# IML-DKFZ/values

Hardware: AMD Instinct MI355X
Metric: uncertainty-volumes/sec (64^3, T=10 MC-dropout) (higher is better)
Workload: dtype f32; 1 GPU; C2: 64^3 1-channel volumes, UNet3D(initial_filter_size=8, 2 classes), T=10 MC-dropout passes + fused softmax/entropy/MI/variance/argmax reduction; dropout=hash bit generator, new seed every step, weights=torch default init, seed 123

## Files before the change

include/values_amd.h:

```cpp
#ifndef VALUES_AMD_H
#define VALUES_AMD_H

#include <stddef.h>
#include <stdint.h>

#ifdef __cplusplus
extern "C" {
#endif

typedef void* vx_stream_t;

enum {
  VX_OK = 0,
  VX_E_NULL = -1,
  VX_E_SHAPE = -2,
  VX_E_DTYPE = -3,
  VX_E_WORKSPACE = -4,
  VX_E_ALIGN = -5
};

enum { VX_F32 = 0, VX_F64 = 1 };
enum { VX_ACT_NONE = 0, VX_ACT_LRELU = 1 , VX_ACT_RELU = 2 };
enum { VX_DROP_NONE = 0, VX_DROP_HASH = 1, VX_DROP_MASK = 2 };

// ... 107 lines not shown
  const float* acc_in;
  int32_t acc_pitch;
  int32_t out_planar, in_planar;
  int32_t products;
} vx_conv3d_args;
int64_t vx_conv3d_upfused_packed_floats(void);
int vx_pack_conv3d_upfused(const float* w1_torch, const float* b1, const float* up_w_torch, const float* up_b, float* packed,
                           vx_stream_t stream);
int vx_conv3d_k3_prologue_ok(int D, int H, int W, int Cin, int Cout);
int vx_conv3d_k3_upfuse_ok(int D, int H, int W, int Cin, int Cout);
int64_t vx_convT_zc16_packed_floats(void);
int vx_pack_convT_zc16(const float* w_torch , float* packed, vx_stream_t stream);
int vx_conv3d_k3_skip_prologue_ok(int D, int H, int W, int Cin, int Cout, int xblk);
int vx_conv3d_k3_acc_ok(int D, int H, int W, int Cin, int Cout);
int vx_conv3d_k3_planar_ok(int D, int H, int W, int Cin, int Cout);
int vx_conv3d_k3_poolfuse_ok(int D, int H, int W, int Cin, int Cout);
int vx_conv3d_k3_presplit_ok(int D, int H, int W, int Cin, int Cout);
int vx_conv3d_k3_poolfin_ok(int Cin, int Cout);
int vx_prenorm_split(float* x, const float* mean, const float* rstd, int N, int64_t nvox, float scale, vx_stream_t stream);
int vx_pool_finish(const float* pool_raw, const uint32_t* pool_flags, const float* mean, const float* rstd, float* out,
                   int out_pitch, int N, int64_t voxels_per_sample, int drop_scale2, vx_stream_t stream);
int vx_pool_finish_z(const float* pool_raw, const uint32_t* pool_flags, const float* mean, const float* rstd, float* out,
                     int out_pitch, int N, int Dp, int64_t plane_voxels, int drop_scale2, vx_stream_t stream);
int vx_conv3d_k3_pool_layout(int D, int H, int W, int Cin, int Cout);
int vx_conv3d_k3_tiles(int D, int H, int W);
int vx_conv3d_k3_tiles_for(int D, int H, int W, int Cout);
int vx_conv3d_k3(const vx_conv3d_args* a, vx_stream_t stream);
int vx_conv3d_k3_head_fusable(int Cin, int Cout);

int vx_conv3d_k3_c1_tiles(int D, int H, int W);
int vx_conv3d_k3_c1(const float* in, const float* w_torch , const float* bias, float* out,
                    int out_pitch, int N, int D, int H, int W, int Cout, int repeat, const int32_t* src,
                    const int32_t* flip, float* stats_partial, vx_stream_t stream);

int vx_pack_input_cl8(const float* in, float* out, int N, int Cin, int D, int H, int W, int repeat, const int32_t* src,
                      const int32_t* flip, vx_stream_t stream);

int vx_instnorm_finalize(const float* stats_partial, int N, int ntiles, int C, int64_t nvox, float eps,
                         float* mean, float* rstd, vx_stream_t stream);

typedef struct vx_norm_args {
  const float* x; int32_t x_pitch;
  const float* mean; const float* rstd;
  float* out; int32_t out_pitch, out_coff;
  float* pool_out; int32_t pool_pitch;
  int32_t N, D, H, W, C;
  int32_t act, drop_mode; uint32_t drop_seed, drop_layer; const uint8_t* drop_mask;
  int32_t out_xblk, out_half;
  int32_t x_xblk, x_half;
  const uint32_t* seed_dev;
  uint32_t* range_flag;
} vx_norm_args;
int vx_norm_act_drop_pool(const vx_norm_args* a, vx_stream_t stream);
typedef struct vx_stat_src {
  const float* stats_partial; int32_t tiles; float eps; int64_t count;
  float* mean_out; float* rstd_out;
} vx_stat_src;
int vx_norm_act_drop_pool_stats(const vx_norm_args* a, const vx_stat_src* st, vx_stream_t stream);
int vx_prenorm_split_stats(float* x, const vx_stat_src* st, int N, int64_t nvox, float scale, vx_stream_t stream);
int vx_zero(void* p, int64_t bytes, vx_stream_t stream);
int vx_pool_finish_z_stats(const float* pool_raw, const uint32_t* pool_flags, const vx_stat_src* st, float* out, int out_pitch,
                           int N, int Dp, int64_t plane_voxels, int drop_scale2, vx_stream_t stream);
int vx_norm_act_drop_pool_bcast(const vx_norm_args* a, int x_repeat, vx_stream_t stream);

typedef struct vx_convT_args {
  const float* in; int32_t in_pitch;
// ... 348 lines not shown
```

values_amd/_lib.py:

```python
from __future__ import annotations

import ctypes as C
import os

_HERE = os.path.dirname(os.path.abspath(__file__))
LIB_PATH = os.environ.get("VX_LIB_PATH") or os.path.join(_HERE, "libvalues_amd.so")

VX_F32, VX_F64 = 0, 1
VX_ACT_NONE, VX_ACT_LRELU, VX_ACT_RELU = 0, 1, 2
VX_DROP_NONE, VX_DROP_HASH, VX_DROP_MASK = 0, 1, 2

_p = C.c_void_p
_i = C.c_int
_i32 = C.c_int32
_u32 = C.c_uint32
_i64 = C.c_int64


class ConvArgs(C.Structure):
    _fields_ = [("in_", _p), ("w_packed", _p), ("bias", _p), ("out", _p),
                ("in_pitch", _i32), ("out_pitch", _i32), ("out_coff", _i32),
                ("N", _i32), ("D", _i32), ("H", _i32), ("W", _i32), ("Cin", _i32), ("Cout", _i32),
                ("act", _i32), ("drop_mode", _i32), ("drop_seed", _u32), ("drop_layer", _u32),
                ("drop_mask", _p), ("stats_partial", _p), ("in_xblk", _i32), ("w_family", _i32),
# ... 203 lines not shown
    "vx_unc_stats_accumulate": (_i, [_p, _i, _i, _i, _i64, _p, _p]),
    "vx_unc_stats_finalize": (_i, [_p, _i, _i, _i, _i64, _p, _p, _p, _p, _p, _p]),
    "vx_softmax_planar": (_i, [_p, _i64, _i, _i64, _p, _p]),
    "vx_one_minus_msr": (_i, [_p, _i, _i, _i64, _p, _p]),
    "vx_one_minus_msr_batched_workspace_bytes": (_i64, [_i, _i]),
    "vx_one_minus_msr_batched": (_i, [C.POINTER(MsrItem), _i, C.POINTER(_p), _i, _p, _i64, _p]),
    "vx_conv3d_k3_packed_floats": (_i64, [_i, _i]),
    "vx_pack_conv3d_k3": (_i, [_p, _p, _i, _i, _p]),
    "vx_convT_k2s2_packed_floats": (_i64, [_i, _i]),
    "vx_pack_convT_k2s2": (_i, [_p, _p, _i, _i, _p]),
    "vx_conv3d_k3_tiles": (_i, [_i, _i, _i]),
    "vx_conv3d_k3_tiles_for": (_i, [_i, _i, _i, _i]),
    "vx_conv3d_k3_head_fusable": (_i, [_i, _i]),
    "vx_conv3d_k3_prologue_ok": (_i, [_i, _i, _i, _i, _i]),
    "vx_conv3d_k3_upfuse_ok": (_i, [_i, _i, _i, _i, _i]),
    "vx_conv3d_k3_poolfuse_ok": (_i, [_i, _i, _i, _i, _i]),
    "vx_conv3d_k3_presplit_ok": (_i, [_i, _i, _i, _i, _i]),
    "vx_conv3d_k3_poolfin_ok": (_i, [_i, _i]),
    "vx_conv3d_upfused_packed_floats": (_i64, []),
    "vx_pack_conv3d_upfused": (_i, [_p, _p, _p, _p, _p, _p]),
    "vx_pool_finish": (_i, [_p, _p, _p, _p, _p, _i, _i, _i64, _i, _p]),
    "vx_pool_finish_z": (_i, [_p, _p, _p, _p, _p, _i, _i, _i, _i64, _i, _p]),
    "vx_conv3d_k3_pool_layout": (_i, [_i, _i, _i, _i, _i]),
    "vx_conv3d_k3_skip_prologue_ok": (_i, [_i, _i, _i, _i, _i, _i]),
    "vx_conv3d_k3_acc_ok": (_i, [_i, _i, _i, _i, _i]),
    "vx_conv3d_k3_planar_ok": (_i, [_i, _i, _i, _i, _i]),
    "vx_convT_zc16_packed_floats": (_i64, []),
    "vx_pack_convT_zc16": (_i, [_p, _p, _p]),
    "vx_prenorm_split": (_i, [_p, _p, _p, _i, _i64, C.c_float, _p]),
    "vx_zero": (_i, [_p, _i64, _p]),
    "vx_conv3d_k3": (_i, [C.POINTER(ConvArgs), _p]),
    "vx_conv3d_k3_c1_tiles": (_i, [_i, _i, _i]),
    "vx_conv3d_k3_c1": (_i, [_p, _p, _p, _p, _i, _i, _i, _i, _i, _i, _i, _p, _p, _p, _p]),
    "vx_pack_input_cl8": (_i, [_p, _p, _i, _i, _i, _i, _i, _i, _p, _p, _p]),
    "vx_instnorm_finalize": (_i, [_p, _i, _i, _i, _i64, C.c_float, _p, _p, _p]),
    "vx_norm_act_drop_pool": (_i, [C.POINTER(NormArgs), _p]),
    "vx_norm_act_drop_pool_bcast": (_i, [C.POINTER(NormArgs), _i, _p]),
    "vx_norm_act_drop_pool_stats": (_i, [C.POINTER(NormArgs), C.POINTER(StatSrc), _p]),
    "vx_prenorm_split_stats": (_i, [_p, C.POINTER(StatSrc), _i, _i64, C.c_float, _p]),
    "vx_pool_finish_z_stats": (_i, [_p, _p, C.POINTER(StatSrc), _p, _i, _i, _i, _i64, _i, _p]),
    "vx_convT_k2s2": (_i, [C.POINTER(ConvTArgs), _p]),
    "vx_conv1x1_ncdhw": (_i, [_p, _i, _p, _p, _p, _i, _i, _i, _i, _i, _i, _p, _p, _p]),
    "vx_unet3d_workspace_bytes": (C.c_size_t, [_i, _i, _i, _i, _i]),
    "vx_unet3d_forward": (_i, [C.POINTER(UNet3DWeights), C.POINTER(UNet3DRun), _p]),
    "vx_unet3d_forward_profiled": (_i, [C.POINTER(UNet3DWeights), C.POINTER(UNet3DRun), _p, _i, C.POINTER(C.c_float),
                                        C.POINTER(C.c_char_p), C.POINTER(_i)]),
    "vx_softmax_accumulate": (_i, [_p, _i, _i, _i, _i, _i, _i, _p, _p, _p, _i, _i, _i, _i, _p]),
    "vx_aleatoric_sample": (_i, [_p, _p, _u32, _i, _i, _i, _i64, _p, _p, _p]),
    "vx_colorize_u8": (_i, [_p, _p, _i64, _p, _i, _p, _p]),
    "vx_fuse_sum": (_i, [C.POINTER(FuseArgs), _p]),
    "vx_tta_views_2d": (_i, [_p, _i, _p, _p, C.POINTER(C.c_float), C.POINTER(C.c_float), C.c_float, _i, _i, _i, _i,
                             C.POINTER(C.c_int32), _p, _p]),
    "vx_count_nonzero_batched_workspace_bytes": (_i64, [_i]),
    "vx_count_nonzero_batched": (_i, [C.POINTER(CountItem), _i, _p, _p, _i64, _p]),
    "vx_select_segments_workspace_bytes": (_i64, [_i]),
    "vx_select_segments": (_i, [C.POINTER(SelectItem), _i, _i64, _p, _p, _p, _i64, _p]),
    "vx_mask_agreement": (_i, [_p, _i, _i, _i64, _p, _p]),
    "vx_mask_agreement_batched": (_i, [_p, _i, _i, _i, _i64, _i, _p, _p]),
    "vx_soft_metric_workspace_bytes": (_i64, [_i, _i]),
    "vx_soft_metric_sums": (_i, [_p, _p, _i, _i, _i64, _p, _p, _p]),
    "vx_soft_metric_batched_workspace_bytes": (_i64, [_i, _i, _i, _i64]),
    "vx_soft_metric_sums_batched": (_i, [_p, _p, _i, _i, _i, _i64, _p, _p, _p]),
    "vx_ssn2d_lowres": (_i, [_p, _i, _p, _i, _p, _u32, _i, _i64, _i, _i, _i, _p, _p, _p]),
    "vx_ssn2d_add_diag": (_i, [_p, _p, _p, _u32, _i, _i, _i64, C.c_float, _p]),
    "vx_softmax_variance": (_i, [_p, _i, _i, _i, _i, _i64, _p, _p]),
    "vx_ssn_sample": (_i, [_p, _p, _p, _u32, _i, _i, _i, _i, _i64, C.c_float, _p, _p]),
# ... 155 lines not shown
```

values_amd/csrc/conv3d_c1.hip:

```cpp
#include "s16_common.h"

template <int COUT>
__global__ __launch_bounds__(256) void conv3d_k3_c1_kernel(const float* __restrict__ in, const float* __restrict__ w,
                                                           const float* __restrict__ bias,
                                                           float* __restrict__ out, int out_pitch, int N, int D, int H, int W,
                                                           int repeat, const int32_t* __restrict__ src,
                                                           const int32_t* __restrict__ flip, float* __restrict__ stats_partial,
                                                           int tiles_x, int tiles_y, int tiles_z) {
  constexpr int TX = 64, TY = 4, TZ = 4;
  constexpr int HX = TX + 2, HY = TY + 2, HZ = TZ + 2;
  __shared__ float s_in[HZ * HY * HX];
  __shared__ __attribute__((aligned(16))) float s_w[27 * COUT];
  __shared__ float s_red[16][COUT][2];

  const int tid = threadIdx.x;
  int t = blockIdx.x;
  const int tx = t % tiles_x; t /= tiles_x;
  const int ty = t % tiles_y; t /= tiles_y;
  const int tz = t % tiles_z; t /= tiles_z;
  const int n = t;
  const int v = src ? src[n] : n / repeat;
  const int f = flip ? flip[n] : 0;
  const int x0 = tx * TX, y0 = ty * TY, z0 = tz * TZ;
  const float* in_v = in + (size_t)v * D * H * W;

  for (int idx = tid; idx < HZ * HY * HX; idx += 256) {
    const int hx = idx % HX, hy = (idx / HX) % HY, hz = idx / (HX * HY);
    int gx = x0 + hx - 1, gy = y0 + hy - 1, gz = z0 + hz - 1;
    float val = 0.f;
    if ((unsigned)gx < (unsigned)W && (unsigned)gy < (unsigned)H && (unsigned)gz < (unsigned)D) {
      if (f & 1) gz = D - 1 - gz;
      if (f & 2) gy = H - 1 - gy;
      if (f & 4) gx = W - 1 - gx;
      val = in_v[((size_t)gz * H + gy) * W + gx];
    }
    s_in[idx] = val;
  }
  for (int idx = tid; idx < 27 * COUT; idx += 256) {
    const int co = idx % COUT, tap = idx / COUT;
    s_w[idx] = w[co * 27 + tap];
  }
  __syncthreads();

  const int lx = tid % TX, ly = tid / TX;
  float acc[TZ][COUT];
#pragma unroll
  for (int z = 0; z < TZ; ++z)
#pragma unroll
    for (int c = 0; c < COUT; ++c) acc[z][c] = bias[c];
#pragma unroll 1
  for (int kk = 0; kk < 9; ++kk) {
    const int ky = kk / 3, kx = kk - 3 * ky;
    float wk[3][COUT];
#pragma unroll
    for (int kz = 0; kz < 3; ++kz)
#pragma unroll
      for (int c = 0; c < COUT; c += 4) {
        const f32x4 w4 = *reinterpret_cast<const f32x4*>(&s_w[(kz * 9 + kk) * COUT + c]);
        wk[kz][c] = w4[0]; wk[kz][c + 1] = w4[1]; wk[kz][c + 2] = w4[2]; wk[kz][c + 3] = w4[3];
      }
    const float* sp = s_in + (ly + ky) * HX + lx + kx;
#pragma unroll
    for (int p = 0; p < HZ; ++p) {
      const float xv = sp[p * HY * HX];
#pragma unroll
      for (int z = 0; z < TZ; ++z) {
        const int kz = p - z;
        if (kz < 0 || kz > 2) continue;
#pragma unroll
        for (int c = 0; c < COUT; ++c) acc[z][c] = fmaf(wk[kz][c], xv, acc[z][c]);
      }
    }
  }

  const int gx = x0 + lx, gy = y0 + ly;
  float ssum[COUT], ssq[COUT];
#pragma unroll
  for (int c = 0; c < COUT; ++c) { ssum[c] = 0.f; ssq[c] = 0.f; }
#pragma unroll
  for (int z = 0; z < TZ; ++z) {
    const int gz = z0 + z;
    const bool valid = gx < W && gy < H && gz < D;
    if (valid) {
      float* o = out + (((size_t)(n * D + gz) * H + gy) * W + gx) * out_pitch;
#pragma unroll
      for (int c = 0; c < COUT; c += 4)
        *reinterpret_cast<f32x4*>(o + c) = (f32x4){acc[z][c], acc[z][c + 1], acc[z][c + 2], acc[z][c + 3]};
#pragma unroll
      for (int c = 0; c < COUT; ++c) { ssum[c] += acc[z][c]; ssq[c] = fmaf(acc[z][c], acc[z][c], ssq[c]); }
    }
  }
  if (stats_partial) {
    const int lane = tid & 63, wave = tid >> 6;
#pragma unroll
    for (int c = 0; c < COUT; ++c) {
      float s = ssum[c], q = ssq[c];
#pragma unroll
      for (int rot = 8; rot >= 1; rot >>= 1) { s += vx_row_ror(s, rot); q += vx_row_ror(q, rot); }
      if ((lane & 15) == 0) { s_red[wave * 4 + (lane >> 4)][c][0] = s; s_red[wave * 4 + (lane >> 4)][c][1] = q; }
    }
    __syncthreads();
    if (tid < COUT) {
      float s = 0.f, q = 0.f;
#pragma unroll
      for (int wv = 0; wv < 16; ++wv) { s += s_red[wv][tid][0]; q += s_red[wv][tid][1]; }
      const int ntiles = tiles_x * tiles_y * tiles_z;
      const int tile = blockIdx.x % ntiles;
      float* dst = stats_partial + (((size_t)n * ntiles + tile) * COUT + tid) * 2;
      dst[0] = s;
      dst[1] = q;
    }
  }
}

extern "C" int vx_conv3d_k3_c1_tiles(int D, int H, int W) { return ((W + 63) / 64) * ((H + 3) / 4) * ((D + 3) / 4); }

extern "C" int vx_conv3d_k3_c1(const float* in, const float* w_torch, const float* bias, float* out, int out_pitch,
                               int N, int D, int H, int W, int Cout, int repeat, const int32_t* src,
                               const int32_t* flip, float* stats_partial, vx_stream_t stream) {
  if (!in || !w_torch || !bias || !out) VX_FAIL(VX_E_NULL, "vx_conv3d_k3_c1: null pointer");
  if (N <= 0 || D <= 0 || H <= 0 || W <= 0) VX_FAIL(VX_E_SHAPE, "vx_conv3d_k3_c1: empty tensor");
  if (repeat <= 0) VX_FAIL(VX_E_SHAPE, "vx_conv3d_k3_c1: repeat must be >= 1");
  if (out_pitch < Cout || out_pitch % 4 || !vx_aligned16(out)) VX_FAIL(VX_E_ALIGN, "vx_conv3d_k3_c1: out pitch/alignment");
  const int tiles_x = (W + 63) / 64, tiles_y = (H + 3) / 4, tiles_z = (D + 3) / 4;
  dim3 grid((unsigned)(tiles_x * tiles_y * tiles_z * N));
  hipStream_t s = (hipStream_t)stream;
#define VX_C1(CO)                                                                                                  \
  vx_note_kernel("conv3d_k3_c1_kernel<" #CO ">");                                                                  \
  hipLaunchKernelGGL(conv3d_k3_c1_kernel<CO>, grid, dim3(256), 0, s, in, w_torch, bias, out, out_pitch, N, D, H, W, \
                     repeat, src, flip, stats_partial, tiles_x, tiles_y, tiles_z)
  switch (Cout) {
    case 8: VX_C1(8); break;
    case 16: VX_C1(16); break;
    case 32: VX_C1(32); break;
    default: VX_FAIL(VX_E_SHAPE, "vx_conv3d_k3_c1: Cout=%d unsupported (8, 16, 32)", Cout);
  }
#undef VX_C1
  VX_CHECK_LAUNCH("vx_conv3d_k3_c1");
  return VX_OK;
}

__global__ __launch_bounds__(256) void pack_input_cl8_kernel(const float* __restrict__ in, float* __restrict__ out, int N, int Cin,
                                                             int D, int H, int W, int repeat, const int32_t* __restrict__ src,
                                                             const int32_t* __restrict__ flip) {
  const int64_t nvox = (int64_t)D * H * W, total = (int64_t)N * nvox;
  for (int64_t i = blockIdx.x * (int64_t)blockDim.x + threadIdx.x; i < total; i += (int64_t)gridDim.x * blockDim.x) {
    const int n = (int)(i / nvox);
    const int64_t v = i - (int64_t)n * nvox;
    int x = (int)(v % W), y = (int)((v / W) % H), z = (int)(v / ((int64_t)W * H));
    const int vol = src ? src[n] : n / repeat;
    const int fl = flip ? flip[n] : 0;
    if (fl & 1) z = D - 1 - z;
    if (fl & 2) y = H - 1 - y;
    if (fl & 4) x = W - 1 - x;
    const float* p = in + ((size_t)vol * Cin) * nvox + ((size_t)z * H + y) * W + x;
    f32x4 lo = {0.f, 0.f, 0.f, 0.f}, hi = {0.f, 0.f, 0.f, 0.f};
#pragma unroll
    for (int c = 0; c < 4; ++c) {
      if (c < Cin) lo[c] = p[(size_t)c * nvox];
      if (c + 4 < Cin) hi[c] = p[(size_t)(c + 4) * nvox];
    }
    reinterpret_cast<f32x4*>(out + (size_t)i * 8)[0] = lo;
    reinterpret_cast<f32x4*>(out + (size_t)i * 8)[1] = hi;
  }
}

extern "C" int vx_pack_input_cl8(const float* in, float* out, int N, int Cin, int D, int H, int W, int repeat,
                                 const int32_t* src, const int32_t* flip, vx_stream_t stream) {
  if (!in || !out) VX_FAIL(VX_E_NULL, "vx_pack_input_cl8: null pointer");
  if (N <= 0 || D <= 0 || H <= 0 || W <= 0 || repeat <= 0) VX_FAIL(VX_E_SHAPE, "vx_pack_input_cl8: empty tensor");
  if (Cin < 1 || Cin > 8) VX_FAIL(VX_E_SHAPE, "vx_pack_input_cl8: in_channels %d (1 .. 8)", Cin);
  if (!vx_aligned16(out)) VX_FAIL(VX_E_ALIGN, "vx_pack_input_cl8: output alignment");
// ... 9 lines not shown
```

values_amd/csrc/lib.cpp:

```cpp
#include <stdarg.h>
#include <stdio.h>
#include <stdlib.h>
#include <string.h>

#include "../../include/values_amd.h"

static thread_local char g_err[512] = "";

void vx_set_error(const char* fmt, ...) {
  va_list ap;
  va_start(ap, fmt);
  vsnprintf(g_err, sizeof(g_err), fmt, ap);
  va_end(ap);
}

static thread_local const char* g_last_kernel = nullptr;
void vx_note_kernel(const char* name) { g_last_kernel = name; }
const char* vx_last_kernel() { return g_last_kernel; }
const char* vx_kname(const char* fmt, ...) {
  char buf[256];
  va_list ap;
  va_start(ap, fmt);
  vsnprintf(buf, sizeof(buf), fmt, ap);
  va_end(ap);
// ... 26 lines not shown
  g_cfg.no_head_fusion = env_int("VX_NO_HEAD_FUSION", 0);
  g_cfg.s16_no_upfuse = env_int("VX_S16_NO_UPFUSE", 0);
  g_cfg.s16_no_poolfuse = env_int("VX_S16_NO_POOLFUSE", 0);
  g_cfg.storage16 = env_int("VX_STORAGE16", 0);
  g_cfg.s16_generic = env_int("VX_S16_GENERIC", 0);
  g_cfg.s16_no_zc16 = env_int("VX_S16_NO_ZC16", 0);
  g_cfg.s16_no_halves = env_int("VX_S16_NO_HALVES", 0);
  g_cfg.s16_no_deep = env_int("VX_S16_NO_DEEP", 0);
  g_cfg.s16_no_l1dma = env_int("VX_S16_NO_L1DMA", 0);
  g_cfg.c2s_no_wide = env_int("VX_C2S_NO_WIDE", 0);
  g_cfg.c2s_no_oct = env_int("VX_C2S_NO_OCT", 0);
}

const vx_config& vx_cfg() {
  std::call_once(g_cfg_once, cfg_from_env);
  return g_cfg;
}

extern "C" int vx_get_config(vx_config* out) {
  if (!out) { vx_set_error("vx_get_config: null"); return VX_E_NULL; }
  *out = vx_cfg();
  return VX_OK;
}

extern "C" int vx_set_config(const vx_config* cfg) {
  if (!cfg) { vx_set_error("vx_set_config: null"); return VX_E_NULL; }
  if (cfg->conv_fp32 < 0 || cfg->conv_fp32 > 2) { vx_set_error("vx_set_config: conv_fp32 %d", cfg->conv_fp32); return VX_E_DTYPE; }
  (void)vx_cfg();
  g_cfg = *cfg;
  return VX_OK;
}

extern "C" const char* vx_last_kernel_name(void) { return g_last_kernel ? g_last_kernel : ""; }
extern "C" int vx_version(void) { return 840;  }
extern "C" const char* vx_last_error_string(void) { return g_err; }
```

values_amd/csrc/unet3d_forward.hip:

```cpp
#include "common.h"
#include <stdlib.h>

extern "C" int vx_conv3d_k3_c1_tiles(int D, int H, int W);

namespace {
struct Level { int D, H, W, C; int64_t nvox; };

struct Plan {
  Level lv[5];
  float *A[4], *B[4], *CAT[4], *P[5], *C0, *C1;
  float *stats, *mean, *rstd;
  float *mean0, *rstd0;
  float *meanS[4], *rstdS[4];
  size_t bytes;
};

static size_t align_up(size_t v) { return (v + 255) & ~(size_t)255; }

static void make_plan(Plan& p, int N, int D, int H, int W, int F, char* base) {
  size_t off = 0;
  auto carve = [&](size_t floats) {
    float* q = base ? (float*)(base + off) : nullptr;
    off += align_up(floats * sizeof(float));
    return q;
  };
  for (int l = 0; l < 5; ++l) {
    p.lv[l].D = D >> l; p.lv[l].H = H >> l; p.lv[l].W = W >> l; p.lv[l].C = F << l;
    p.lv[l].nvox = (int64_t)p.lv[l].D * p.lv[l].H * p.lv[l].W;
  }
  for (int l = 0; l < 4; ++l) {
    const size_t e = (size_t)N * p.lv[l].nvox * p.lv[l].C;
    p.A[l] = carve(e);
    p.B[l] = carve(e);
    p.CAT[l] = carve(2 * e);
  }
  p.P[0] = nullptr;
// ... 43 lines not shown
thread_local char g_prof_labels[Prof::MAXL][192];
}

#define VX_TRY(expr)            \
  do {                          \
    int rc_ = (expr);           \
    if (rc_ != VX_OK) return rc_; \
  } while (0)

#define VX_STEP(label, expr)                                                       \
  do {                                                                             \
    Prof* pf_ = g_prof;                                                            \
    if (pf_ && pf_->n < Prof::MAXL) { vx_note_kernel(nullptr); (void)hipEventRecord(pf_->ev[2 * pf_->n], pf_->s); }  \
    int rc_ = (expr);                                                              \
    if (rc_ != VX_OK) return rc_;                                                  \
    if (pf_ && pf_->n < Prof::MAXL) {                                              \
      (void)hipEventRecord(pf_->ev[2 * pf_->n + 1], pf_->s);                             \
      pf_->kernel[pf_->n] = vx_last_kernel();                                      \
      pf_->name[pf_->n++] = (label);                                               \
    }                                                                              \
  } while (0)

namespace {
int xblk_of(int W) { return W % 4 == 0 ? 4 : (W % 2 == 0 ? 2 : 1); }

struct Flow {
  bool inorm;
  int ich;
  int rep;
  bool shared;
  bool fuse_head;
  bool pre[4];
  bool presplit;
  bool skip_raw[4];
  bool pooled[4];
  bool poolfin1;
  bool halves[4];
  bool fuse_up;
  bool fuse_up1;
  bool split_out[4];
  bool planar1;
  bool st16;
  int products_c12, products_e11, products_e12;
};

Flow decide_flow(const vx_unet3d_weights* w, const vx_unet3d_run* r, const Plan& p) {
  const vx_config& cfg = vx_cfg();
  const int F = w->F, dm = r->drop_mode;
  const Level* lv = p.lv;
  const bool hashed = dm != VX_DROP_MASK;
  Flow f = {};
  f.inorm = !w->no_instancenorm;
  f.ich = w->in_channels > 1 ? w->in_channels : 1;
  f.rep = r->repeat > 0 ? r->repeat : 1;
  f.shared = !r->src && !r->flip && f.rep > 1 && r->N % f.rep == 0;
  f.fuse_head = w->num_classes <= 4 && vx_conv3d_k3_head_fusable(F, F) && !cfg.no_head_fusion;
  f.pre[0] = hashed && !cfg.s16_no_prenorm && F == 8 && f.inorm && vx_conv3d_k3_prologue_ok(lv[0].D, lv[0].H, lv[0].W, F, F);
  for (int l = 1; l < 4; ++l)
    f.pre[l] = f.inorm && hashed && !cfg.s16_no_prenorm && vx_conv3d_k3_prologue_ok(lv[l].D, lv[l].H, lv[l].W, lv[l].C, lv[l].C);
  f.presplit = f.shared && f.pre[0] && vx_conv3d_k3_presplit_ok(lv[0].D, lv[0].H, lv[0].W, F, F);
  f.skip_raw[0] = f.pre[0] && cfg.s16_skip_raw && vx_conv3d_k3_prologue_ok(lv[0].D, lv[0].H, lv[0].W, 2 * F, F);
  f.pooled[0] = f.skip_raw[0] && vx_conv3d_k3_poolfuse_ok(lv[0].D, lv[0].H, lv[0].W, F, F);
  f.poolfin1 = f.pooled[0] && vx_conv3d_k3_poolfin_ok(F, 2 * F);
  for (int l = 1; l < 4; ++l) {
    const Level& L = lv[l];
    f.skip_raw[l] = f.pooled[l] = f.inorm && hashed && !cfg.s16_no_prenorm && cfg.s16_skip_raw &&
                                  vx_conv3d_k3_pool_layout(L.D, L.H, L.W, L.C, L.C) == 2 &&
                                  vx_conv3d_k3_skip_prologue_ok(L.D, L.H, L.W, 2 * L.C, L.C, xblk_of(L.W));
  }
  f.halves[1] = f.skip_raw[1] && lv[1].C == 16 && w->split_w[0] && w->split_w[1] && !cfg.s16_no_halves &&
                w->split_family == vx_conv3d_k3_family(16, 16) && vx_conv3d_k3_acc_ok(lv[1].D, lv[1].H, lv[1].W, 16, 16);
  f.fuse_up = hashed && F == 8 && vx_conv3d_k3_upfuse_ok(lv[0].D, lv[0].H, lv[0].W, 2 * F, F);
  f.fuse_up1 = f.halves[1] && w->up3_zc16 && hashed && vx_conv3d_k3_upfuse_ok(lv[1].D, lv[1].H, lv[1].W, 16, 16) == 2;
  f.split_out[1] = f.fuse_up;
  f.split_out[2] = f.fuse_up1;
  f.planar1 = f.fuse_up1 && !cfg.s16_no_l1dma && vx_conv3d_k3_planar_ok(lv[1].D, lv[1].H, lv[1].W, 16, 16);
  f.st16 = cfg.storage16 && dm == VX_DROP_HASH && F == 8 && f.fuse_head && cfg.conv_fp32 == 0 &&
           vx_conv3d_k3_prologue_ok(lv[0].D, lv[0].H, lv[0].W, F, F);
  const bool one = f.st16 && cfg.storage16 == 2;
  f.products_c12 = one && f.presplit && f.pooled[0];
  f.products_e11 = one && f.skip_raw[0] && f.fuse_up && w->up_fused;
  f.products_e12 = one;
  return f;
}
}

extern "C" int vx_unet3d_forward(const vx_unet3d_weights* w, const vx_unet3d_run* r, vx_stream_t stream) {
  if (!w || !r) VX_FAIL(VX_E_NULL, "vx_unet3d_forward: null argument");
  if (!r->x || !r->logits || !r->workspace) VX_FAIL(VX_E_NULL, "vx_unet3d_forward: null tensor/workspace");
  const int N = r->N, D = r->D, H = r->H, W = r->W, F = w->F, NC = w->num_classes;
  if (N <= 0 || D <= 0 || H <= 0 || W <= 0) VX_FAIL(VX_E_SHAPE, "vx_unet3d_forward: empty batch");
  if (D % 16 || H % 16 || W % 16)
    VX_FAIL(VX_E_SHAPE, "vx_unet3d_forward: spatial size (%d,%d,%d) must be divisible by 16 (4 poolings; InstanceNorm "
            "needs > 1 voxel at the 8x level)", D, H, W);
  if (F != 8 && F != 16 && F != 32) VX_FAIL(VX_E_SHAPE, "vx_unet3d_forward: initial_filter_size %d unsupported (8,16,32)", F);
  if (NC <= 0) VX_FAIL(VX_E_SHAPE, "vx_unet3d_forward: num_classes %d", NC);
  if (r->drop_mode < 0 || r->drop_mode > 2) VX_FAIL(VX_E_DTYPE, "vx_unet3d_forward: drop_mode %d", r->drop_mode);
  if ((((uintptr_t)r->workspace) & 255u) != 0) VX_FAIL(VX_E_ALIGN, "vx_unet3d_forward: workspace must be 256-byte aligned");
  for (int i = 0; i < 18; ++i)
// ... 59 lines not shown
  };
  auto pool_flags = [&](int l) {
    const size_t maxima = l == 0 ? (size_t)N * p.lv[1].nvox * 8 : (size_t)N * (p.lv[l].nvox / 4) * p.lv[l].C;
    return reinterpret_cast<uint32_t*>(p.B[l] + maxima);
  };
  auto first_conv = [&](float* out, int n_out, int rep, float* stats) -> int {
    const Level& L = p.lv[0];
    if (f.ich == 1)
      return vx_conv3d_k3_c1(r->x, w->conv_w[0], w->conv_b[0], out, L.C, n_out, L.D, L.H, L.W, L.C, rep, r->src, r->flip, stats, stream);
    VX_TRY(vx_pack_input_cl8(r->x, p.B[0], n_out, f.ich, L.D, L.H, L.W, rep, r->src, r->flip, stream));
    vx_conv3d_args a = conv_args(0, L, 8, L.C, stats);
    a.N = n_out; a.in = p.B[0]; a.in_pitch = 8; a.out = out; a.out_pitch = L.C;
    return vx_conv3d_k3(&a, stream);
  };

  static const char* kConv[18] = {"contr_1_1", "contr_1_2", "contr_2_1", "contr_2_2", "contr_3_1", "contr_3_2",
                                  "contr_4_1", "contr_4_2", "center.0", "center.2", "expand_4_1", "expand_4_2",
                                  "expand_3_1", "expand_3_2", "expand_2_1", "expand_2_2", "expand_1_1", "expand_1_2"};
  static const char* kNorm[8] = {"norm:contr_1_1", "norm:contr_1_2", "norm:contr_2_1", "norm:contr_2_2",
                                 "norm:contr_3_1", "norm:contr_3_2", "norm:contr_4_1", "norm:contr_4_2"};
  static const char* kFin[8] = {"finalize:contr_1_1", "finalize:contr_1_2", "finalize:contr_2_1", "finalize:contr_2_2",
                                "finalize:contr_3_1", "finalize:contr_3_2", "finalize:contr_4_1", "finalize:contr_4_2"};
  static const char* kPoolFin[4] = {"poolfin:contr_1_2", "poolfin:contr_2_2", "poolfin:contr_3_2", "poolfin:contr_4_2"};
  static const char* kUp[4] = {"center.4", "upscale4", "upscale3", "upscale2"};
  float* const out1 = f.shared && !f.skip_raw[0] ? p.CAT[0] : p.A[0];
  const int fan = f.shared ? f.rep : 1;
  for (int l = 0; l < 4; ++l) {
    const Level& L = p.lv[l];
    const int C = L.C;
    const int ntiles = vx_conv3d_k3_tiles_for(L.D, L.H, L.W, C);
    if (l == 0) {
      const int n1 = N / fan;
      const int ntiles1 = f.ich == 1 ? vx_conv3d_k3_c1_tiles(L.D, L.H, L.W) : ntiles;
      VX_STEP(kConv[0], first_conv(out1, n1, f.shared ? 1 : f.rep, f.inorm ? p.stats : nullptr));
      if (f.inorm) VX_STEP(kFin[0], vx_instnorm_finalize(p.stats, n1, ntiles1, C, L.nvox, 1e-5f, p.mean, p.rstd, stream));
      if (f.presplit)
        VX_STEP("presplit:contr_1_1", vx_prenorm_split(out1, p.mean, p.rstd, n1, L.nvox, dm == VX_DROP_HASH ? 2.f : 1.f, stream));
      if (!f.pre[0]) {
        vx_norm_args n = norm_args(out1, C, L, 0, f.inorm);
        n.out = p.A[0]; n.out_pitch = C;
        VX_STEP(kNorm[0], vx_norm_act_drop_pool_bcast(&n, fan, stream));
      }
    } else {
      vx_conv3d_args a = conv_args(2 * l, L, C / 2, C, f.inorm ? p.stats : nullptr);
      a.in = p.P[l]; a.in_pitch = C / 2; a.out = p.A[l]; a.out_pitch = C;
      if (!f.inorm) set_drop(a, VX_ACT_LRELU, 2 * l);
      if (l == 1 && f.poolfin1) {
        a.in = p.B[0]; a.in_pool_flags = pool_flags(0);
        set_pre(a, 1, 1, p.mean0, p.rstd0);
      }
      VX_STEP(l == 1 && f.poolfin1 ? "poolfin+contr_2_1" : kConv[2 * l], vx_conv3d_k3(&a, stream));
      if (f.inorm) {
        VX_STEP(kFin[2 * l], vx_instnorm_finalize(p.stats, N, ntiles, C, L.nvox, 1e-5f, p.mean, p.rstd, stream));
        if (!f.pre[l]) {
          vx_norm_args n = norm_args(p.A[l], C, L, 2 * l, true);
          n.out = p.A[l]; n.out_pitch = C;
          VX_STEP(kNorm[2 * l], vx_norm_act_drop_pool_bcast(&n, 1, stream));
        }
      }
    }
    if (!f.inorm) {
      vx_conv3d_args a = conv_args(2 * l + 1, L, C, C, nullptr);
      a.in = p.A[l]; a.in_pitch = C; a.out = p.B[l]; a.out_pitch = C;
      set_drop(a, VX_ACT_LRELU, 2 * l + 1);
      VX_STEP(kConv[2 * l + 1], vx_conv3d_k3(&a, stream));
      vx_norm_args n = norm_args(p.B[l], C, L, -1, false);
      n.act = VX_ACT_NONE;
      n.out = p.CAT[l]; n.out_pitch = 2 * C; n.out_coff = C; n.out_xblk = xblk_of(L.W); n.pool_out = p.P[l + 1];
      VX_STEP(kNorm[2 * l + 1], vx_norm_act_drop_pool_bcast(&n, 1, stream));
// ... 141 lines not shown
```

Baseline: 3921 volumes/s.

## Recompute first 1-channel conv to fuse stats pass and prenorm split

The first conv (Cin=1) now runs twice: once computing only instance-norm statistics without writing output, then again applying normalize, leaky-ReLU, dropout scale and fp16 hi/lo split directly in its epilogue. This drops the raw 8-channel write, its re-read and the separate prenorm-split kernel, in exchange for redoing cheap single-channel conv arithmetic. The kernel also gains a persistent-grid mode with register prefetch of the next tile, an optional paired-z tile and LDS-staged coalesced row stores for 8-channel output.

```diff
diff --git a/include/values_amd.h b/include/values_amd.h
--- a/include/values_amd.h
+++ b/include/values_amd.h
@@ -163,6 +163,11 @@
 int vx_conv3d_k3_c1(const float* in, const float* w_torch , const float* bias, float* out,
                     int out_pitch, int N, int D, int H, int W, int Cout, int repeat, const int32_t* src,
                     const int32_t* flip, float* stats_partial, vx_stream_t stream);
+int vx_conv3d_k3_c1_stats(const float* in, const float* w_torch, const float* bias, int N, int D, int H, int W, int Cout,
+                          int repeat, const int32_t* src, const int32_t* flip, float* stats_partial, vx_stream_t stream);
+int vx_conv3d_k3_c1_presplit(const float* in, const float* w_torch, const float* bias, const float* mean, const float* rstd,
+                             float scale, float* out, int N, int D, int H, int W, int Cout, int repeat, const int32_t* src,
+                             const int32_t* flip, vx_stream_t stream);
 
 int vx_pack_input_cl8(const float* in, float* out, int N, int Cin, int D, int H, int W, int repeat, const int32_t* src,
                       const int32_t* flip, vx_stream_t stream);
diff --git a/values_amd/_lib.py b/values_amd/_lib.py
--- a/values_amd/_lib.py
+++ b/values_amd/_lib.py
@@ -259,6 +259,8 @@
     "vx_conv3d_k3": (_i, [C.POINTER(ConvArgs), _p]),
     "vx_conv3d_k3_c1_tiles": (_i, [_i, _i, _i]),
     "vx_conv3d_k3_c1": (_i, [_p, _p, _p, _p, _i, _i, _i, _i, _i, _i, _i, _p, _p, _p, _p]),
+    "vx_conv3d_k3_c1_stats": (_i, [_p, _p, _p, _i, _i, _i, _i, _i, _i, _p, _p, _p, _p]),
+    "vx_conv3d_k3_c1_presplit": (_i, [_p, _p, _p, _p, _p, C.c_float, _p, _i, _i, _i, _i, _i, _i, _p, _p, _p]),
     "vx_pack_input_cl8": (_i, [_p, _p, _i, _i, _i, _i, _i, _i, _p, _p, _p]),
     "vx_instnorm_finalize": (_i, [_p, _i, _i, _i, _i64, C.c_float, _p, _p, _p]),
     "vx_norm_act_drop_pool": (_i, [C.POINTER(NormArgs), _p]),
diff --git a/values_amd/csrc/conv3d_c1.hip b/values_amd/csrc/conv3d_c1.hip
--- a/values_amd/csrc/conv3d_c1.hip
+++ b/values_amd/csrc/conv3d_c1.hip
@@ -1,143 +1,299 @@
 #include "s16_common.h"
 
-template <int COUT>
-__global__ __launch_bounds__(256) void conv3d_k3_c1_kernel(const float* __restrict__ in, const float* __restrict__ w,
+enum { C1_RAW = 0, C1_STATS = 1, C1_SPLIT = 2 };
+
+template <int COUT, int MODE, int ZP> struct C1Geom {
+  static constexpr int WAVES = COUT == 8 && (MODE != 0 || ZP == 1) ? 4 : 1;
+};
+
+template <int COUT, int MODE, int ZP>
+__global__ __launch_bounds__(256, (C1Geom<COUT, MODE, ZP>::WAVES)) void conv3d_k3_c1_kernel(const float* __restrict__ in, const float* __restrict__ w,
                                                            const float* __restrict__ bias,
                                                            float* __restrict__ out, int out_pitch, int N, int D, int H, int W,
                                                            int repeat, const int32_t* __restrict__ src,
                                                            const int32_t* __restrict__ flip, float* __restrict__ stats_partial,
+                                                           const float* __restrict__ mean, const float* __restrict__ rstd, float scale,
                                                            int tiles_x, int tiles_y, int tiles_z) {
   constexpr int TX = 64, TY = 4, TZ = 4;
-  constexpr int HX = TX + 2, HY = TY + 2, HZ = TZ + 2;
+  constexpr int CZ = TZ * ZP;
+  constexpr int HX = TX + 2, HY = TY + 2, HZ = CZ + 2;
+  static_assert(MODE != C1_SPLIT || COUT == 8, "the pre-split layout is that of an 8-channel tensor");
   __shared__ float s_in[HZ * HY * HX];
   __shared__ __attribute__((aligned(16))) float s_w[27 * COUT];
-  __shared__ float s_red[16][COUT][2];
+  __shared__ float s_red[MODE == C1_SPLIT ? 1 : ZP][16][COUT][2];
+  constexpr bool ROWST = COUT == 8 && MODE != C1_STATS;
+  __shared__ __attribute__((aligned(16))) float s_out[ROWST ? 4 : 1][ROWST ? TX * 8 : 4];
 
   const int tid = threadIdx.x;
-  int t = blockIdx.x;
-  const int tx = t % tiles_x; t /= tiles_x;
-  const int ty = t % tiles_y; t /= tiles_y;
-  const int tz = t % tiles_z; t /= tiles_z;
-  const int n = t;
-  const int v = src ? src[n] : n / repeat;
-  const int f = flip ? flip[n] : 0;
-  const int x0 = tx * TX, y0 = ty * TY, z0 = tz * TZ;
-  const float* in_v = in + (size_t)v * D * H * W;
-
-  for (int idx = tid; idx < HZ * HY * HX; idx += 256) {
-    const int hx = idx % HX, hy = (idx / HX) % HY, hz = idx / (HX * HY);
-    int gx = x0 + hx - 1, gy = y0 + hy - 1, gz = z0 + hz - 1;
+  const int lane = tid & 63, wave = __builtin_amdgcn_readfirstlane(tid >> 6);
+  const int lx = tid % TX, ly = tid / TX;
+  const int tiles_zg = (tiles_z + ZP - 1) / ZP;
+  const int items = tiles_x * tiles_y * tiles_zg * N;
+
+  struct Item { int tx, ty, tzg, n, x0, y0, z0, f; const float* in_v; };
+  auto decode = [&](int item) {
+    Item it;
+    int t = item;
+    it.tx = t % tiles_x; t /= tiles_x;
+    it.ty = t % tiles_y; t /= tiles_y;
+    it.tzg = t % tiles_zg; t /= tiles_zg;
+    it.n = t;
+    const int v = src ? src[it.n] : it.n / repeat;
+    it.f = flip ? flip[it.n] : 0;
+    it.x0 = it.tx * TX; it.y0 = it.ty * TY; it.z0 = it.tzg * CZ;
+    it.in_v = in + (size_t)v * D * H * W;
+    return it;
+  };
+  auto fetch = [&](const Item& it, int row, int hx) -> float {
+    const int hz = row / HY, hy = row - hz * HY;
+    int gx = it.x0 + hx - 1, gy = it.y0 + hy - 1, gz = it.z0 + hz - 1;
     float val = 0.f;
     if ((unsigned)gx < (unsigned)W && (unsigned)gy < (unsigned)H && (unsigned)gz < (unsigned)D) {
-      if (f & 1) gz = D - 1 - gz;
-      if (f & 2) gy = H - 1 - gy;
-      if (f & 4) gx = W - 1 - gx;
-      val = in_v[((size_t)gz * H + gy) * W + gx];
-    }
-    s_in[idx] = val;
-  }
+      if (it.f & 1) gz = D - 1 - gz;
+      if (it.f & 2) gy = H - 1 - gy;
+      if (it.f & 4) gx = W - 1 - gx;
+      val = it.in_v[((size_t)gz * H + gy) * W + gx];
+    }
+    return val;
+  };
+  constexpr int RW = HZ * HY / 4;
+  static_assert(HZ * HY % 4 == 0 && 2 * HZ * HY <= 256, "rows per wave");
+  float pre[RW], pre_x = 0.f;
+  auto prefetch = [&](int item) {
+    const Item it = decode(item);
+#pragma unroll
+    for (int i = 0; i < RW; ++i) pre[i] = fetch(it, wave + 4 * i, lane);
+    if (tid < 2 * HZ * HY) pre_x = fetch(it, tid >> 1, TX + (tid & 1));
+  };
+
   for (int idx = tid; idx < 27 * COUT; idx += 256) {
     const int co = idx % COUT, tap = idx / COUT;
     s_w[idx] = w[co * 27 + tap];
   }
-  __syncthreads();
-
-  const int lx = tid % TX, ly = tid / TX;
-  float acc[TZ][COUT];
-#pragma unroll
-  for (int z = 0; z < TZ; ++z)
-#pragma unroll
-    for (int c = 0; c < COUT; ++c) acc[z][c] = bias[c];
+  if ((int)blockIdx.x < items) prefetch(blockIdx.x);
+  for (int item = blockIdx.x; item < items; item += gridDim.x) {
+    const Item cur = decode(item);
+    const int tx = cur.tx, ty = cur.ty, tzg = cur.tzg, n = cur.n, x0 = cur.x0, y0 = cur.y0, z0 = cur.z0;
+#pragma unroll
+    for (int i = 0; i < RW; ++i) s_in[(wave + 4 * i) * HX + lane] = pre[i];
+    if (tid < 2 * HZ * HY) s_in[(tid >> 1) * HX + TX + (tid & 1)] = pre_x;
+    __syncthreads();
+    if (item + (int)gridDim.x < items) prefetch(item + gridDim.x);
+
+    float acc[CZ][COUT];
+#pragma unroll
+    for (int z = 0; z < CZ; ++z)
+#pragma unroll
+      for (int c = 0; c < COUT; ++c) acc[z][c] = bias[c];
 #pragma unroll 1
-  for (int kk = 0; kk < 9; ++kk) {
-    const int ky = kk / 3, kx = kk - 3 * ky;
-    float wk[3][COUT];
-#pragma unroll
-    for (int kz = 0; kz < 3; ++kz)
-#pragma unroll
-      for (int c = 0; c < COUT; c += 4) {
-        const f32x4 w4 = *reinterpret_cast<const f32x4*>(&s_w[(kz * 9 + kk) * COUT + c]);
-        wk[kz][c] = w4[0]; wk[kz][c + 1] = w4[1]; wk[kz][c + 2] = w4[2]; wk[kz][c + 3] = w4[3];
-      }
-    const float* sp = s_in + (ly + ky) * HX + lx + kx;
-#pragma unroll
-    for (int p = 0; p < HZ; ++p) {
-      const float xv = sp[p * HY * HX];
-#pragma unroll
-      for (int z = 0; z < TZ; ++z) {
-        const int kz = p - z;
-        if (kz < 0 || kz > 2) continue;
-#pragma unroll
-        for (int c = 0; c < COUT; ++c) acc[z][c] = fmaf(wk[kz][c], xv, acc[z][c]);
-      }
-    }
-  }
-
-  const int gx = x0 + lx, gy = y0 + ly;
-  float ssum[COUT], ssq[COUT];
-#pragma unroll
-  for (int c = 0; c < COUT; ++c) { ssum[c] = 0.f; ssq[c] = 0.f; }
-#pragma unroll
-  for (int z = 0; z < TZ; ++z) {
-    const int gz = z0 + z;
-    const bool valid = gx < W && gy < H && gz < D;
-    if (valid) {
-      float* o = out + (((size_t)(n * D + gz) * H + gy) * W + gx) * out_pitch;
-#pragma unroll
-      for (int c = 0; c < COUT; c += 4)
-        *reinterpret_cast<f32x4*>(o + c) = (f32x4){acc[z][c], acc[z][c + 1], acc[z][c + 2], acc[z][c + 3]};
-#pragma unroll
-      for (int c = 0; c < COUT; ++c) { ssum[c] += acc[z][c]; ssq[c] = fmaf(acc[z][c], acc[z][c], ssq[c]); }
-    }
-  }
-  if (stats_partial) {
-    const int lane = tid & 63, wave = tid >> 6;
-#pragma unroll
-    for (int c = 0; c < COUT; ++c) {
-      float s = ssum[c], q = ssq[c];
-#pragma unroll
-      for (int rot = 8; rot >= 1; rot >>= 1) { s += vx_row_ror(s, rot); q += vx_row_ror(q, rot); }
-      if ((lane & 15) == 0) { s_red[wave * 4 + (lane >> 4)][c][0] = s; s_red[wave * 4 + (lane >> 4)][c][1] = q; }
+    for (int kk = 0; kk < 9; ++kk) {
+      const int ky = kk / 3, kx = kk - 3 * ky;
+      float wk[3][COUT];
+#pragma unroll
+      for (int kz = 0; kz < 3; ++kz)
+#pragma unroll
+        for (int c = 0; c < COUT; c += 4) {
+          const f32x4 w4 = *reinterpret_cast<const f32x4*>(&s_w[(kz * 9 + kk) * COUT + c]);
+          wk[kz][c] = w4[0]; wk[kz][c + 1] = w4[1]; wk[kz][c + 2] = w4[2]; wk[kz][c + 3] = w4[3];
+        }
+      const float* sp = s_in + (ly + ky) * HX + lx + kx;
+#pragma unroll
+      for (int p = 0; p < HZ; ++p) {
+        const float xv = sp[p * HY * HX];
+#pragma unroll
+        for (int z = 0; z < CZ; ++z) {
+          const int kz = p - z;
+          if (kz < 0 || kz > 2) continue;
+#pragma unroll
+          for (int c = 0; c < COUT; ++c) acc[z][c] = fmaf(wk[kz][c], xv, acc[z][c]);
+        }
+      }
+    }
+
+    const int gx = x0 + lx, gy = y0 + ly;
+    auto store_row = [&](int gz, const f32x4 p0, const f32x4 p1) {
+      f32x4* so = reinterpret_cast<f32x4*>(s_out[wave]);
+      __builtin_amdgcn_wave_barrier();
+      so[2 * lane] = p0;
+      so[2 * lane + 1] = p1;
+      __builtin_amdgcn_wave_barrier();
+      const f32x4 a = so[lane], b = so[64 + lane];
+      __builtin_amdgcn_wave_barrier();
+      if (gy < H && gz < D) {
+        f32x4* o = reinterpret_cast<f32x4*>(out + (((size_t)(n * D + gz) * H + gy) * W + x0) * 8);
+        if (x0 + (lane >> 1) < W) o[lane] = a;
+        if (x0 + 32 + (lane >> 1) < W) o[64 + lane] = b;
+      }
+    };
+    if constexpr (MODE == C1_SPLIT) {
+      f32x4 mu[2], sc[2];
+#pragma unroll
+      for (int q = 0; q < 2; ++q) {
+        mu[q] = *reinterpret_cast<const f32x4*>(mean + (size_t)n * 8 + q * 4);
+        sc[q] = *reinterpret_cast<const f32x4*>(rstd + (size_t)n * 8 + q * 4);
+#pragma unroll
+        for (int j = 0; j < 4; ++j) sc[q][j] = sc[q][j] * scale;
+      }
+#pragma unroll
+      for (int z = 0; z < CZ; ++z) {
+        const int gz = z0 + z;
+        f32x4 pc[2];
+#pragma unroll
+        for (int q = 0; q < 2; ++q) {
+          f32x4 y = {acc[z][4 * q], acc[z][4 * q + 1], acc[z][4 * q + 2], acc[z][4 * q + 3]};
+#pragma unroll
+          for (int j = 0; j < 4; ++j) {
+            const float tt = (y[j] - mu[q][j]) * sc[q][j];
+            y[j] = fmaxf(tt, 0.01f * tt);
+          }
+          f16x4 hi, lo;
+          vx_split4(y, hi, lo);
+          f32x4 piece;
+          piece[0] = __builtin_bit_cast(float, (f16x2){hi[0], hi[1]});
+          piece[1] = __builtin_bit_cast(float, (f16x2){hi[2], hi[3]});
+          piece[2] = __builtin_bit_cast(float, (f16x2){lo[0], lo[1]});
+          piece[3] = __builtin_bit_cast(float, (f16x2){lo[2], lo[3]});
+          pc[q] = piece;
+        }
+        store_row(gz, pc[0], pc[1]);
+      }
+    } else {
+      const bool stats = MODE == C1_STATS || stats_partial;
+#pragma unroll
+      for (int zp = 0; zp < ZP; ++zp) {
+        float ssum[COUT], ssq[COUT];
+#pragma unroll
+        for (int c = 0; c < COUT; ++c) { ssum[c] = 0.f; ssq[c] = 0.f; }
+#pragma unroll
+        for (int zz = 0; zz < TZ; ++zz) {
+          const int z = zp * TZ + zz, gz = z0 + z;
+          const bool valid = gx < W && gy < H && gz < D;
+          if constexpr (ROWST) {
+            if (out_pitch == 8) {
+              store_row(gz, (f32x4){acc[z][0], acc[z][1], acc[z][2], acc[z][3]}, (f32x4){acc[z][4], acc[z][5], acc[z][6], acc[z][7]});
+            }
+          }
+          if (valid) {
+            if (MODE == C1_RAW && !(ROWST && out_pitch == 8)) {
+              float* o = out + (((size_t)(n * D + gz) * H + gy) * W + gx) * out_pitch;
+#pragma unroll
+              for (int c = 0; c < COUT; c += 4)
+                *reinterpret_cast<f32x4*>(o + c) = (f32x4){acc[z][c], acc[z][c + 1], acc[z][c + 2], acc[z][c + 3]};
+            }
+#pragma unroll
+            for (int c = 0; c < COUT; ++c) { ssum[c] += acc[z][c]; ssq[c] = fmaf(acc[z][c], acc[z][c], ssq[c]); }
+          }
+        }
+        if (stats) {
+#pragma unroll
+          for (int c = 0; c < COUT; ++c) {
+            float s = ssum[c], q = ssq[c];
+#pragma unroll
+            for (int rot = 8; rot >= 1; rot >>= 1) { s += vx_row_ror(s, rot); q += vx_row_ror(q, rot); }
+            if ((lane & 15) == 0) { s_red[zp][wave * 4 + (lane >> 4)][c][0] = s; s_red[zp][wave * 4 + (lane >> 4)][c][1] = q; }
+          }
+        }
+      }
+      if (stats) {
+        __syncthreads();
+        const int zp = tid / COUT, c = tid - zp * COUT, tz = tzg * ZP + zp;
+        if (tid < ZP * COUT && tz < tiles_z) {
+          float s = 0.f, q = 0.f;
+#pragma unroll
+          for (int wv = 0; wv < 16; ++wv) { s += s_red[zp][wv][c][0]; q += s_red[zp][wv][c][1]; }
+          const int ntiles = tiles_x * tiles_y * tiles_z;
+          const int tile = (tz * tiles_y + ty) * tiles_x + tx;
+          float* dst = stats_partial + (((size_t)n * ntiles + tile) * COUT + c) * 2;
+          dst[0] = s;
+          dst[1] = q;
+        }
+      }
     }
     __syncthreads();
-    if (tid < COUT) {
-      float s = 0.f, q = 0.f;
-#pragma unroll
-      for (int wv = 0; wv < 16; ++wv) { s += s_red[wv][tid][0]; q += s_red[wv][tid][1]; }
-      const int ntiles = tiles_x * tiles_y * tiles_z;
-      const int tile = blockIdx.x % ntiles;
-      float* dst = stats_partial + (((size_t)n * ntiles + tile) * COUT + tid) * 2;
-      dst[0] = s;
-      dst[1] = q;
-    }
   }
 }
 
 extern "C" int vx_conv3d_k3_c1_tiles(int D, int H, int W) { return ((W + 63) / 64) * ((H + 3) / 4) * ((D + 3) / 4); }
+
+namespace {
+struct C1Args {
+  const float *in, *w, *bias; float* out; int out_pitch, N, D, H, W, repeat; const int32_t *src, *flip; float* stats_partial;
+  const float *mean, *rstd; float scale;
+};
+
+template <int CO, int MODE, int ZP> void c1_go(const C1Args& a, hipStream_t s) {
+  const int tiles_x = (a.W + 63) / 64, tiles_y = (a.H + 3) / 4, tiles_z = (a.D + 3) / 4;
+  const int64_t items = (int64_t)tiles_x * tiles_y * ((tiles_z + ZP - 1) / ZP) * a.N;
+  int64_t blocks = items;
+  if (MODE == C1_RAW) {
+    static int per_cu = 0;
+    if (per_cu == 0) {
+      int v = 0;
+      const hipError_t e = hipOccupancyMaxActiveBlocksPerMultiprocessor(&v, conv3d_k3_c1_kernel<CO, MODE, ZP>, 256, 0);
+      per_cu = e == hipSuccess && v > 0 ? v : 1;
+    }
+    const int64_t resident = (int64_t)vx_cu_count() * per_cu;
+    if (blocks > resident) blocks = resident;
+  }
+  static const char* kname = vx_kname("conv3d_k3_c1_kernel<%d, %d, %d>", CO, MODE, ZP);
+  vx_note_kernel(kname);
+  hipLaunchKernelGGL((conv3d_k3_c1_kernel<CO, MODE, ZP>), dim3((unsigned)blocks), dim3(256), 0, s, a.in, a.w, a.bias, a.out, a.out_pitch,
+                     a.N, a.D, a.H, a.W, a.repeat, a.src, a.flip, a.stats_partial, a.mean, a.rstd, a.scale, tiles_x, tiles_y, tiles_z);
+}
+
+template <int MODE> int c1_mode(const C1Args& a, int Cout, bool pair, hipStream_t s, const char* who) {
+  switch (Cout) {
+    case 8: if (pair) c1_go<8, MODE, 2>(a, s); else c1_go<8, MODE, 1>(a, s); break;
+    case 16: if (MODE == C1_SPLIT) VX_FAIL(VX_E_SHAPE, "%s: Cout=%d unsupported (8)", who, Cout); c1_go<16, MODE == C1_SPLIT ? C1_STATS : MODE, 1>(a, s); break;
+    case 32: if (MODE == C1_SPLIT) VX_FAIL(VX_E_SHAPE, "%s: Cout=%d unsupported (8)", who, Cout); c1_go<32, MODE == C1_SPLIT ? C1_STATS : MODE, 1>(a, s); break;
+    default: VX_FAIL(VX_E_SHAPE, "%s: Cout=%d unsupported (8, 16, 32)", who, Cout);
+  }
+  return VX_OK;
+}
+
+int c1_launch(int mode, const float* in, const float* w_torch, const float* bias, float* out, int out_pitch, int N, int D, int H,
+              int W, int Cout, int repeat, const int32_t* src, const int32_t* flip, float* stats_partial, const float* mean,
+              const float* rstd, float scale, hipStream_t s, const char* who) {
+  if (N <= 0 || D <= 0 || H <= 0 || W <= 0) VX_FAIL(VX_E_SHAPE, "%s: empty tensor", who);
+  if (repeat <= 0) VX_FAIL(VX_E_SHAPE, "%s: repeat must be >= 1", who);
+  if ((int64_t)N * D * H * W >= (1ll << 31)) VX_FAIL(VX_E_SHAPE, "%s: more than 2^31 voxels", who);
+  const int64_t tiles = (int64_t)((W + 63) / 64) * ((H + 3) / 4) * ((D + 3) / 4) * N;
+  const bool pair = tiles / 2 >= 2 * (int64_t)vx_cu_count();
+  const C1Args a = {in, w_torch, bias, out, out_pitch, N, D, H, W, repeat, src, flip, stats_partial, mean, rstd, scale};
+  int rc;
+  if (mode == C1_SPLIT) rc = c1_mode<C1_SPLIT>(a, Cout, pair, s, who);
+  else if (mode == C1_STATS) rc = c1_mode<C1_STATS>(a, Cout, pair, s, who);
+  else rc = c1_mode<C1_RAW>(a, Cout, pair, s, who);
+  if (rc != VX_OK) return rc;
+  VX_CHECK_LAUNCH(who);
+  return VX_OK;
+}
+}
 
 extern "C" int vx_conv3d_k3_c1(const float* in, const float* w_torch, const float* bias, float* out, int out_pitch,
                                int N, int D, int H, int W, int Cout, int repeat, const int32_t* src,
                                const int32_t* flip, float* stats_partial, vx_stream_t stream) {
   if (!in || !w_torch || !bias || !out) VX_FAIL(VX_E_NULL, "vx_conv3d_k3_c1: null pointer");
-  if (N <= 0 || D <= 0 || H <= 0 || W <= 0) VX_FAIL(VX_E_SHAPE, "vx_conv3d_k3_c1: empty tensor");
-  if (repeat <= 0) VX_FAIL(VX_E_SHAPE, "vx_conv3d_k3_c1: repeat must be >= 1");
   if (out_pitch < Cout || out_pitch % 4 || !vx_aligned16(out)) VX_FAIL(VX_E_ALIGN, "vx_conv3d_k3_c1: out pitch/alignment");
-  const int tiles_x = (W + 63) / 64, tiles_y = (H + 3) / 4, tiles_z = (D + 3) / 4;
-  dim3 grid((unsigned)(tiles_x * tiles_y * tiles_z * N));
-  hipStream_t s = (hipStream_t)stream;
-#define VX_C1(CO)                                                                                                  \
-  vx_note_kernel("conv3d_k3_c1_kernel<" #CO ">");                                                                  \
-  hipLaunchKernelGGL(conv3d_k3_c1_kernel<CO>, grid, dim3(256), 0, s, in, w_torch, bias, out, out_pitch, N, D, H, W, \
-                     repeat, src, flip, stats_partial, tiles_x, tiles_y, tiles_z)
-  switch (Cout) {
-    case 8: VX_C1(8); break;
-    case 16: VX_C1(16); break;
-    case 32: VX_C1(32); break;
-    default: VX_FAIL(VX_E_SHAPE, "vx_conv3d_k3_c1: Cout=%d unsupported (8, 16, 32)", Cout);
-  }
-#undef VX_C1
-  VX_CHECK_LAUNCH("vx_conv3d_k3_c1");
-  return VX_OK;
+  return c1_launch(C1_RAW, in, w_torch, bias, out, out_pitch, N, D, H, W, Cout, repeat, src, flip, stats_partial, nullptr, nullptr,
+                   0.f, (hipStream_t)stream, "vx_conv3d_k3_c1");
+}
+
+extern "C" int vx_conv3d_k3_c1_stats(const float* in, const float* w_torch, const float* bias, int N, int D, int H, int W,
+                                     int Cout, int repeat, const int32_t* src, const int32_t* flip, float* stats_partial,
+                                     vx_stream_t stream) {
+  if (!in || !w_torch || !bias || !stats_partial) VX_FAIL(VX_E_NULL, "vx_conv3d_k3_c1_stats: null pointer");
+  return c1_launch(C1_STATS, in, w_torch, bias, nullptr, 0, N, D, H, W, Cout, repeat, src, flip, stats_partial, nullptr, nullptr,
+                   0.f, (hipStream_t)stream, "vx_conv3d_k3_c1_stats");
+}
+
+extern "C" int vx_conv3d_k3_c1_presplit(const float* in, const float* w_torch, const float* bias, const float* mean,
+                                        const float* rstd, float scale, float* out, int N, int D, int H, int W, int Cout,
+                                        int repeat, const int32_t* src, const int32_t* flip, vx_stream_t stream) {
+  if (!in || !w_torch || !bias || !mean || !rstd || !out) VX_FAIL(VX_E_NULL, "vx_conv3d_k3_c1_presplit: null pointer");
+  if (!vx_aligned16(out) || !vx_aligned16(mean) || !vx_aligned16(rstd)) VX_FAIL(VX_E_ALIGN, "vx_conv3d_k3_c1_presplit: alignment");
+  return c1_launch(C1_SPLIT, in, w_torch, bias, out, 8, N, D, H, W, Cout, repeat, src, flip, nullptr, mean, rstd, scale,
+                   (hipStream_t)stream, "vx_conv3d_k3_c1_presplit");
 }
 
 __global__ __launch_bounds__(256) void pack_input_cl8_kernel(const float* __restrict__ in, float* __restrict__ out, int N, int Cin,
diff --git a/values_amd/csrc/lib.cpp b/values_amd/csrc/lib.cpp
--- a/values_amd/csrc/lib.cpp
+++ b/values_amd/csrc/lib.cpp
@@ -82,5 +82,5 @@
 }
 
 extern "C" const char* vx_last_kernel_name(void) { return g_last_kernel ? g_last_kernel : ""; }
-extern "C" int vx_version(void) { return 840;  }
+extern "C" int vx_version(void) { return 841;  }
 extern "C" const char* vx_last_error_string(void) { return g_err; }
diff --git a/values_amd/csrc/unet3d_forward.hip b/values_amd/csrc/unet3d_forward.hip
--- a/values_amd/csrc/unet3d_forward.hip
+++ b/values_amd/csrc/unet3d_forward.hip
@@ -2,6 +2,11 @@
 #include <stdlib.h>
 
 extern "C" int vx_conv3d_k3_c1_tiles(int D, int H, int W);
+extern "C" int vx_conv3d_k3_c1_stats(const float* in, const float* w_torch, const float* bias, int N, int D, int H, int W, int Cout,
+                                     int repeat, const int32_t* src, const int32_t* flip, float* stats_partial, vx_stream_t stream);
+extern "C" int vx_conv3d_k3_c1_presplit(const float* in, const float* w_torch, const float* bias, const float* mean,
+                                        const float* rstd, float scale, float* out, int N, int D, int H, int W, int Cout, int repeat,
+                                        const int32_t* src, const int32_t* flip, vx_stream_t stream);
 
 namespace {
 struct Level { int D, H, W, C; int64_t nvox; };
@@ -111,6 +116,7 @@
   bool fuse_head;
   bool pre[4];
   bool presplit;
+  bool recompute1;
   bool skip_raw[4];
   bool pooled[4];
   bool poolfin1;
@@ -134,16 +140,17 @@
   f.rep = r->repeat > 0 ? r->repeat : 1;
   f.shared = !r->src && !r->flip && f.rep > 1 && r->N % f.rep == 0;
   f.fuse_head = w->num_classes <= 4 && vx_conv3d_k3_head_fusable(F, F) && !cfg.no_head_fusion;
-  f.pre[0] = hashed && !cfg.s16_no_prenorm && F == 8 && f.inorm && vx_conv3d_k3_prologue_ok(lv[0].D, lv[0].H, lv[0].W, F, F);
+  f.pre[0] = hashed && !(cfg.s16_no_prenorm & 1) && F == 8 && f.inorm && vx_conv3d_k3_prologue_ok(lv[0].D, lv[0].H, lv[0].W, F, F);
   for (int l = 1; l < 4; ++l)
-    f.pre[l] = f.inorm && hashed && !cfg.s16_no_prenorm && vx_conv3d_k3_prologue_ok(lv[l].D, lv[l].H, lv[l].W, lv[l].C, lv[l].C);
+    f.pre[l] = f.inorm && hashed && !(cfg.s16_no_prenorm & 1) && vx_conv3d_k3_prologue_ok(lv[l].D, lv[l].H, lv[l].W, lv[l].C, lv[l].C);
   f.presplit = f.shared && f.pre[0] && vx_conv3d_k3_presplit_ok(lv[0].D, lv[0].H, lv[0].W, F, F);
+  f.recompute1 = f.presplit && f.ich == 1 && !(cfg.s16_no_prenorm & 2);
   f.skip_raw[0] = f.pre[0] && cfg.s16_skip_raw && vx_conv3d_k3_prologue_ok(lv[0].D, lv[0].H, lv[0].W, 2 * F, F);
   f.pooled[0] = f.skip_raw[0] && vx_conv3d_k3_poolfuse_ok(lv[0].D, lv[0].H, lv[0].W, F, F);
   f.poolfin1 = f.pooled[0] && vx_conv3d_k3_poolfin_ok(F, 2 * F);
   for (int l = 1; l < 4; ++l) {
     const Level& L = lv[l];
-    f.skip_raw[l] = f.pooled[l] = f.inorm && hashed && !cfg.s16_no_prenorm && cfg.s16_skip_raw &&
+    f.skip_raw[l] = f.pooled[l] = f.inorm && hashed && !(cfg.s16_no_prenorm & 1) && cfg.s16_skip_raw &&
                                   vx_conv3d_k3_pool_layout(L.D, L.H, L.W, L.C, L.C) == 2 &&
                                   vx_conv3d_k3_skip_prologue_ok(L.D, L.H, L.W, 2 * L.C, L.C, xblk_of(L.W));
   }
@@ -269,9 +276,15 @@
     if (l == 0) {
       const int n1 = N / fan;
       const int ntiles1 = f.ich == 1 ? vx_conv3d_k3_c1_tiles(L.D, L.H, L.W) : ntiles;
-      VX_STEP(kConv[0], first_conv(out1, n1, f.shared ? 1 : f.rep, f.inorm ? p.stats : nullptr));
+      if (f.recompute1)
+        VX_STEP("stats:contr_1_1", vx_conv3d_k3_c1_stats(r->x, w->conv_w[0], w->conv_b[0], n1, L.D, L.H, L.W, C, 1, nullptr, nullptr, p.stats, stream));
+      else
+        VX_STEP(kConv[0], first_conv(out1, n1, f.shared ? 1 : f.rep, f.inorm ? p.stats : nullptr));
       if (f.inorm) VX_STEP(kFin[0], vx_instnorm_finalize(p.stats, n1, ntiles1, C, L.nvox, 1e-5f, p.mean, p.rstd, stream));
-      if (f.presplit)
+      if (f.recompute1)
+        VX_STEP("contr_1_1+presplit", vx_conv3d_k3_c1_presplit(r->x, w->conv_w[0], w->conv_b[0], p.mean, p.rstd, dm == VX_DROP_HASH ? 2.f : 1.f,
+                                                               out1, n1, L.D, L.H, L.W, C, 1, nullptr, nullptr, stream));
+      else if (f.presplit)
         VX_STEP("presplit:contr_1_1", vx_prenorm_split(out1, p.mean, p.rstd, n1, L.nvox, dm == VX_DROP_HASH ? 2.f : 1.f, stream));
       if (!f.pre[0]) {
         vx_norm_args n = norm_args(out1, C, L, 0, f.inorm);
```

Result: no change. 3935 volumes/s (median of 6 runs) (+0.3%).
